# RemoteSensingTools/vSmartMOM.jl

Hardware: AMD Instinct MI355X
Metric: spectral-points/s (whole node) for rt_run, O2-A band (higher is better)
Workload: dtype f64; 1 GPU; C2: O2-A 759-770 nm, nStokes=3, Nquad=20 (N=60), 40 layers, 10000 spectral points/GPU, m=0..2, Rayleigh+synthetic O2 absorption, Lambertian 0.15; ranks=1, collective_backend=none (1 rank), N=60, layers=40, points_per_gpu=10000, fourier_moments=3

## Files before the change

### include/vsmartmom_hip.h

```cpp
#ifndef VSMARTMOM_HIP_H
#define VSMARTMOM_HIP_H

#include <stddef.h>
#include <stdint.h>

#ifdef __cplusplus
extern "C" {
#endif

typedef enum vsm_status {
  VSM_OK = 0,
  VSM_ERR_INVALID_ARG = 1,
  VSM_ERR_UNSUPPORTED = 2,
  VSM_ERR_HIP = 3,
  VSM_ERR_NO_DEVICE = 4
} vsm_status;

typedef enum vsm_iface {
  VSM_IFACE_00 = 0,
  VSM_IFACE_01 = 1,
  VSM_IFACE_10 = 2,
  VSM_IFACE_11 = 3
} vsm_iface;

// ... 336 lines not shown
size_t vsm_run_workspace_bytes_f32(int N, int n_stokes, int S, int nm, const int* coupling_h);
int vsm_run_create_f64(const vsm_quad_f64* q, int S, int nm, const int* m_h, const int* coupling_h, void* workspace,
                       size_t workspace_bytes, vsm_run** run);
int vsm_run_create_f32(const vsm_quad_f32* q, int S, int nm, const int* m_h, const int* coupling_h, void* workspace,
                       size_t workspace_bytes, vsm_run** run);
int vsm_run_create_ex_f64(const vsm_quad_f64* q, int S, int nm, const int* m_h, const int* coupling_h, void* workspace,
                          size_t workspace_bytes, unsigned flags, vsm_run** run);
int vsm_run_create_ex_f32(const vsm_quad_f32* q, int S, int nm, const int* m_h, const int* coupling_h, void* workspace,
                          size_t workspace_bytes, unsigned flags, vsm_run** run);
int vsm_run_create_view_f64(const vsm_quad_f64* q, int S, int nm, const int* m_h, const int* coupling_h, void* workspace,
                            size_t workspace_bytes, unsigned flags, int nrows, const int* rows_h, vsm_run** run);
int vsm_run_create_view_f32(const vsm_quad_f32* q, int S, int nm, const int* m_h, const int* coupling_h, void* workspace,
                            size_t workspace_bytes, unsigned flags, int nrows, const int* rows_h, vsm_run** run);
int vsm_run_create_view_f64(const vsm_quad_f64* q, int S, int nm, const int* m_h, const int* coupling_h, void* workspace,
                            size_t workspace_bytes, unsigned flags, int nrows, const int* rows_h, vsm_run** run);
int vsm_run_create_view_f32(const vsm_quad_f32* q, int S, int nm, const int* m_h, const int* coupling_h, void* workspace,
                            size_t workspace_bytes, unsigned flags, int nrows, const int* rows_h, vsm_run** run);
int vsm_run_layer_f64(vsm_run* run, int ndoubl, const double* dtau, const double* varpi, const double* tau_sum,
                      const double* F0, int ncomp, const double* const* Zpp, const double* const* Zmp, long long z_stride,
                      const double* fcomp, int toa, const int* layer_coupling_h, void* stream);
int vsm_run_layer_f32(vsm_run* run, int ndoubl, const float* dtau, const float* varpi, const float* tau_sum,
                      const float* F0, int ncomp, const float* const* Zpp, const float* const* Zmp, long long z_stride,
                      const float* fcomp, int toa, const int* layer_coupling_h, void* stream);
int vsm_run_export_f64(vsm_run* run, const vsm_composite_f64* comps, void* stream);
int vsm_run_export_f32(vsm_run* run, const vsm_composite_f32* comps, void* stream);
int vsm_run_import_f64(vsm_run* run, const vsm_composite_f64* comps, void* stream);
int vsm_run_import_f32(vsm_run* run, const vsm_composite_f32* comps, void* stream);
int vsm_run_zw_tail(vsm_run* run);
int vsm_run_view_rows(vsm_run* run, int nrows, const int* rows_h);
int vsm_run_view_block(const vsm_run* run, int block, int* im, int* n, int* nv, int* local_rows);
int vsm_run_view_rows(vsm_run* run, int nrows, const int* rows_h);
int vsm_run_view_block(const vsm_run* run, int block, int* im, int* n, int* nv, int* local_rows);
int vsm_run_destroy(vsm_run* run);
int vsm_stokes_coupling_f64(int N, int n_stokes, int nblocks, const double* Zpp, const double* Zmp, int* mask_d, void* stream);
int vsm_stokes_coupling_f32(int N, int n_stokes, int nblocks, const float* Zpp, const float* Zmp, int* mask_d, void* stream);

typedef struct vsm_added_rs_f64 {
  double *ier_mp, *iet_pp, *ier_pm, *iet_mm;
  double *ieJ0_p, *ieJ0_m;
  int K;
  int reserved;
} vsm_added_rs_f64;
typedef struct vsm_added_rs_f32 {
  float *ier_mp, *iet_pp, *ier_pm, *iet_mm;
  float *ieJ0_p, *ieJ0_m;
  int K;
// ... 174 lines not shown
```

### vsmartmom.jl_amd/_lib.py

```python
from __future__ import annotations

import ctypes as C
import os

_HERE = os.path.dirname(os.path.abspath(__file__))
LIB_PATH = os.environ.get("VSM_LIB_PATH") or os.path.join(_HERE, "lib", "libvsmartmom_hip.so")


class VSMError(RuntimeError):
    pass


class vsm_quad_f64(C.Structure):
    _fields_ = [("mu", C.c_void_p), ("wt", C.c_void_p), ("N", C.c_int), ("n_stokes", C.c_int),
                ("i_mu0", C.c_int), ("mu0", C.c_double)]


class vsm_quad_f32(C.Structure):
    _fields_ = [("mu", C.c_void_p), ("wt", C.c_void_p), ("N", C.c_int), ("n_stokes", C.c_int),
                ("i_mu0", C.c_int), ("mu0", C.c_float)]


class vsm_added(C.Structure):
    _fields_ = [("r_mp", C.c_void_p), ("t_pp", C.c_void_p), ("r_pm", C.c_void_p), ("t_mm", C.c_void_p),
# ... 104 lines not shown
    "vsm_doubling_inelastic_work_elems": (_SZ, [_I, _I, _I]),
    "vsm_interaction_inelastic_work_elems": (_SZ, [_I, _I, _I]),
    "vsm_elemental_inelastic_rrs_{T}": (_I, [_P, _I, _I, _I, _P, _P, _P, _P, _P, _P]),
    "vsm_doubling_inelastic_rrs_{T}": (_I, [_I, _I, _I, _I, _P, _P, _P, _P, _P, _P]),
    "vsm_interaction_inelastic_rrs_{T}": (_I, [_I, _I, _I, _P, _P, _P, _P, _P, _P, _P]),
    "vsm_copy_added_to_composite_ie_{T}": (_I, [_I, _I, _P, _P, _P]),
    "vsm_postprocess_vza_ie_{T}": (_I, [_I, _I, _I, _I, _I, _P, _P, _P, _P, _P, _P, _P]),
    "vsm_ss_column_{T}": (_I, [_P, _I, _I, _I, _P, _P, _P, _P, _P, _P, _P, _P, _P, _P, _I, _P, _P, _P, _P, _P, _P, _P]),
    "vsm_ss_column_lin_{T}": (_I, [_P, _I, _I, _I, _I, _I, _I, _I, _I, _P, _P, _P, _P, _P, _P, _P, _P, _P, _P, _I, _P, _P, _P, _P, _P, _P, _P,
                                   _P, _P, _I, _P, _P, _P, _P, _P]),
    "vsm_ss_column_rrs_{T}": (_I, [_P, _I, _I, _I, _I, _P, _P, _P, _P, _P, _P, _P, _P, _I, _I, _P, _P, _P, _P, _P]),
    "vsm_exact_ss_path1_{T}": (_I, [_I, _I, _I, _I, _I, _P, _P, _P, _P, "{R}", _P, _P, _P]),
    "vsm_exact_ss_path2_{T}": (_I, [_I, _I, _I, _I, _I, _P, _P, _I, _P, "{R}", _P, _P, _P]),
    "vsm_exact_ss_path34_{T}": (_I, [_I, _I, _I, _I, _I, _P, _P, _P, _P, _P, _P, _P, _P, "{R}", _P, _P, _P, _P]),
    "vsm_exact_ss_jac12_{T}": (_I, [_I, _I, _I, _I, _I, _P, _P, _P, _P, _I, _P, "{R}", _P, _P, _P, _P, _P, _P, _P]),
    "vsm_run_supported": (_I, [_I, _I, _I]),
    "vsm_run_workspace_bytes": (_SZ, [_I, _I, _I, _I, _P]),
    "vsm_run_supported_f32": (_I, [_I, _I, _I]),
    "vsm_run_workspace_bytes_f32": (_SZ, [_I, _I, _I, _I, _P]),
    "vsm_run_create_{T}": (_I, [_P, _I, _I, _P, _P, _P, _SZ, _P]),
    "vsm_run_create_ex_{T}": (_I, [_P, _I, _I, _P, _P, _P, _SZ, C.c_uint, _P]),
    "vsm_run_create_view_{T}": (_I, [_P, _I, _I, _P, _P, _P, _SZ, C.c_uint, _I, _P, _P]),
    "vsm_run_layer_{T}": (_I, [_P, _I, _P, _P, _P, _P, _I, _P, _P, _LL, _P, _I, _P, _P]),
    "vsm_run_export_{T}": (_I, [_P, _P, _P]),
    "vsm_run_import_{T}": (_I, [_P, _P, _P]),
    "vsm_run_zw_tail": (_I, [_P]),
    "vsm_run_view_rows": (_I, [_P, _I, _P]),
    "vsm_run_view_block": (_I, [_P, _I, _P, _P, _P, _P]),
    "vsm_run_destroy": (_I, [_P]),
    "vsm_stokes_coupling_{T}": (_I, [_I, _I, _I, _P, _P, _P, _P]),
    "vsm_level_radiance_work_elems": (_SZ, [_I, _I]),
    "vsm_level_radiance_{T}": (_I, [_I, _I, _I, _I, _P, _P, _P, _P, _P, _LL, _P, _P, _P, _P, _P, _P, _P]),
    "vsm_level_radiance_oplevel_{T}": (_I, [_I, _I, _I, _I, _P, _P, _P, _P, _P, _LL, _P, _P, _P, _P, _P, _P, _P]),
    "vsm_level_radiance_src_{T}": (_I, [_I, _I, _I, _I, _P, _P, _P, _I, _P, _P, _LL, _P, _P, _P, _P, _P, _P, _P]),
    "vsm_level_radiance_ie_{T}": (_I, [_I, _I, _I, _I, _P, _I, _P, _P, _P, _P, _LL, _P, _P, _P, _P, _P, _P, _P, _P, _P, _P, _P]),
    "vsm_level_radiance_lin_{T}": (_I, [_I, _I, _I, _I, _I, _I, _P, _P, _P, _P, _LL, _P, _P, _P, _LL, _P, _P, _LL, _LL, _P, _P, _P, _P, _P,
                                        _P]),
    "vsm_test_lds_mm_{T}": (_I, [_I, _I, _P, _P, _P, _P]),
    "vsm_test_lds_inv_{T}": (_I, [_I, _I, _P, _P, _I, _P, _P]),
    "vsm_test_poison_lds": (_I, [_P]),
}


def exported_symbols():
    out = []
    for name in _SIGS:
# ... 91 lines not shown
```

### vsmartmom.jl_amd/core_rt.py

```python
from __future__ import annotations

import ctypes as C
import dataclasses
import math
import os
from dataclasses import dataclass
from typing import List, Optional

import numpy as np
import torch

from . import _lib
from . import host_model as H
from .architectures import GPU, CPU, architecture, array_type, devi, synchronize_if_gpu, to_host

IFACE = {"00": 0, "01": 1, "10": 2, "11": 3}
MOMENT_BATCH = 4
MOMENT_BATCH_MAX = 24
MOMENT_BATCHING = True
THERMAL_FUSION = True
NATIVE_RUN = True
NATIVE_SOURCES_ONLY = True
NATIVE_VIEW_ROWS = True
VIEW_ROWS_MAX = 16
NATIVE_ZW_TAIL = True
NATIVE_DROPIN = True
REFERENCE_ORDER = False


def _require_gpu(arch):
    if not isinstance(arch, GPU):
        raise _lib.VSMError("vsmartmom.jl_amd provides the MI355X path only; architecture %r has no compute path here "
                            "(no CPU fallback by design)" % (arch,))
    if not torch.cuda.is_available():
        raise _lib.VSMError("no MI355X visible to HIP (torch.cuda.is_available() is False)")
    if arch.device_index != torch.cuda.current_device():
        raise _lib.VSMError("architecture GPU(%d) is not the current HIP device (%d): one process per GPU -- call "
                            "torch.cuda.set_device(%d) first" % (arch.device_index, torch.cuda.current_device(),
                                                                 arch.device_index))


def _torch_dtype(FT):
    return torch.float64 if np.dtype(FT) == np.float64 else torch.float32


def _stream_ptr():
    return C.c_void_p(torch.cuda.current_stream().cuda_stream)

# ... 246 lines not shown

_work_cache = {}


def layer_forward_multi_(tau_sum, dtau, F0, props_list, ms, ndoubl: int, dq: DeviceQuad, toa: bool, comps, added: AddedLayer):
    nm = len(ms)
    p0 = props_list[0]
    q, a = dq.cstruct(), added.cstruct()
    dtype = comps[0].dtype
    carr = (type(comps[0].cstruct()) * nm)(*[c.cstruct() for c in comps])
    marr = (C.c_int * nm)(*[int(m) for m in ms])
    zpp = (C.c_void_p * nm)(*[p.Zpp.data_ptr() for p in props_list])
    zmp = (C.c_void_p * nm)(*[p.Zmp.data_ptr() for p in props_list])
    ncomp = 0 if p0.fcomp is None else int(p0.fcomp.shape[1])
    _lib.call("vsm_layer_forward_multi", dtype, C.byref(q), comps[0].nSpec, nm, marr, ndoubl, _ptr(dtau), _ptr(p0.varpi),
              _ptr(tau_sum), _ptr(F0), ncomp, zpp, zmp, 0 if ncomp else p0.z_stride, _ptr(p0.fcomp), None, 1 if toa else 0,
              carr, C.byref(a), _stream_ptr())


def run_layer_native_(run, nm: int, ndoubl: int, dtau, varpi, tau_sum, F0, ncomp: int, zpp, zmp, z_stride: int, fcomp, toa: bool,
                      layer_coupling=None, dtype=torch.float64):
    _lib.call("vsm_run_layer", dtype, run, ndoubl, _ptr(dtau), _ptr(varpi), _ptr(tau_sum), _ptr(F0), ncomp, zpp, zmp, z_stride,
              _ptr(fcomp), 1 if toa else 0, layer_coupling, _stream_ptr())


def interaction_(scattering_interface: str, comp: CompositeLayer, added: AddedLayer, oplevel: bool = False,
                 work: Optional[torch.Tensor] = None):
    a, c = added.cstruct(), comp.cstruct()
    N, S = comp.N, comp.nSpec
    fused = (scattering_interface == "11" and not oplevel
             and N <= _lib.lib().vsm_fused_max_n(8 if comp.dtype == torch.float64 else 4))
    if not fused and work is None:
        key = (N, S, comp.dtype, str(comp.R_mp.device))
        work = _work_cache.get(key)
        if work is None:
            _work_cache.clear()
            work = _lib.poison(torch.empty(int(_lib.lib().vsm_interaction_work_elems(N, S)), dtype=comp.dtype, device=comp.R_mp.device))
            _work_cache[key] = work
    name = "vsm_interaction_oplevel" if oplevel else "vsm_interaction"
    _lib.call(name, comp.dtype, IFACE[scattering_interface], N, S, C.byref(c), C.byref(a), _ptr(work), _stream_ptr())


_phi_cache = {}


def brdf_azimuth_quadrature(arch, FT):
# ... 517 lines not shown
            return self.R_SFI, self.T_SFI
        self.added.j0_p.zero_()
        eps2 = 2 * np.finfo(FT).eps
        has_noscat = any(ly["props"].max_tau_varpi <= eps2 for ly in self.moments[0]["layers"])
        sequential = trace is not None or not MOMENT_BATCHING or has_noscat or REFERENCE_ORDER
        want = max(MOMENT_BATCH, min(MOMENT_BATCH_MAX, 4096 // max(self.S, 1)))
        nb = 1 if sequential else min(want, len(self.moments))
        while len(self._composites) < nb:
            self._composites.append(make_composite_layer(FT, self.arch, (self.N, self.N), self.S))
        native = self._native_moments() if trace is None and not has_noscat and not REFERENCE_ORDER else set()
        walk_src = streams is None and trace is None and not has_noscat
        if getattr(self, "_view_rows", None) is None:
            self._view_rows = view_rows_of(pol, model.vza, self.qp)
        view_rows = self._view_rows if streams is None else None
        for c in self._composites:
            c._sources_only = walk_src and REFERENCE_ORDER
            c._view_rows = view_rows if c._sources_only else None
        for g0 in range(0, len(self.moments), nb):
            group = self.moments[g0:g0 + nb]
            comps = self._composites[:len(group)]
            nat = [k for k in range(len(group)) if (g0 + k) in native]
            if nat:
                self._run_layers_native([group[k] for k in nat], [comps[k] for k in nat], sources_only=streams is None,
                                        view_rows=view_rows)
            rest = [k for k in range(len(group)) if (g0 + k) not in native]
            group_l, comps_l = [group[k] for k in rest], [comps[k] for k in rest]
            for iz in range(self.Nz if rest else 0):
                ly0 = group_l[0]["layers"][iz]
                if len(group_l) > 1 and ly0["props"].max_tau_varpi > eps2 and (iz == 0 or ly0["iface"] == "11"):
                    layer_forward_multi_(ly0["tau_sum"], ly0["dtau"], self.F0, [mom["layers"][iz]["props"] for mom in group_l],
                                         [mom["m"] for mom in group_l], ly0["nd"], self.dq, iz == 0, comps_l, self.added)
                    continue
                for mom, comp in zip(group_l, comps_l):
                    ly = mom["layers"][iz]
                    rt_kernel_(pol, self.added, comp, ly["props"], ly["iface"], ly["tau_sum"], mom["m"], self.dq,
                               self.arch, iz + 1, self.F0, FT, model.numerics, dtau=ly["dtau"], ndoubl=ly["nd"], trace=trace,
                               work=self.work, keep_added=has_noscat)
            for mom, comp in zip(group, comps):
                m = mom["m"]
                weight = FT(0.5 / math.pi) if m == 0 else FT(1.0 / math.pi)
                create_surface_layer_(model.surface, self.added_surface, m, self.dq, mom["tau_sum_surface"], rho=mom["rho"])
                interaction_(mom["iface_surface"], comp, self.added_surface, work=self.work)
                if self.compute_hdrf:
                    interaction_hdrf_(pol, comp, self.added_surface, m, self.dq, model.vza, model.vaz, self.qp, float(weight),
                                      self.hdr_J, self.hdr, self.bhr_uw, self.bhr_dw)
                postprocessing_vza_(pol, comp, model.vza, model.vaz, self.qp, m, float(weight), self.R_SFI, self.T_SFI)
                thermal_pass = self.thermal_B is not None and (m == 0 or (m == 1 and self._thermal_carry))
# ... 3 lines not shown
                    Jm, Jp = comp.J0_m.clone(), comp.J0_p.clone()
                    if thermal_pass:
                        Jm += self._th_comp.J0_m
                        Jp += self._th_comp.J0_p
                    streams.append(dict(m=m, weight=float(weight), R_mp=comp.R_mp.clone(), T_pp=comp.T_pp.clone(), J0_m=Jm, J0_p=Jp))
        for c in self._composites:
            c._sources_only = False
            c._view_rows = None
        if isinstance(model.surface, H.CoxMunkSurface) and self.ss_correction:
            apply_ss_correction_(self.R_SFI, model.surface, pol, model.vza, model.vaz, self.qp.mu0,
                                 self.moments[-1]["tau_sum_surface"], model.m_max, self.arch, FT)
        return self.R_SFI, self.T_SFI

    def _native_moments(self):
        if not NATIVE_RUN or getattr(self, "coupling", None) is None or not self.moments:
            return set()
        eps2 = 2 * np.finfo(self.FT).eps
        for iz, ly in enumerate(self.moments[0]["layers"]):
            p = ly["props"]
            if p.max_tau_varpi <= eps2 or (iz > 0 and ly["iface"] != "11") or (p.fcomp is not None and p.fcomp.shape[1] > 4):
                return set()
        return {i for i, mom in enumerate(self.moments) if run_supported(self.dt, self.N, self.pol.n, int(self.coupling[mom["m"]]))}

    def _run_layers_native(self, group, comps, sources_only: bool = True, export_at=None, view_rows=None):
        L = _lib.lib()
        nm, N, S, ns = len(group), self.N, self.S, self.pol.n
        marr = (C.c_int * nm)(*[int(mom["m"]) for mom in group])
        carr = (C.c_int * nm)(*[int(self.coupling[mom["m"]]) for mom in group])
        nbytes = run_workspace_bytes(self.dt, N, ns, S, nm, carr)
        ws = getattr(self, "_native_ws", None)
        if ws is None or ws.numel() * 8 < nbytes:
            ws = self._native_ws = _lib.poison(torch.empty(max(nbytes // 8, 2), dtype=torch.float64, device=self.dev))
        q = self.dq.cstruct()
        run = C.c_void_p()
        run_create_(self.dt, q, S, nm, marr, carr, ws, nbytes, sources_only, view_rows, run)
        try:
            if NATIVE_ZW_TAIL and not torch.cuda.is_current_stream_capturing():
                _lib.check(L.vsm_run_zw_tail(run))
            for iz in range(self.Nz):
                ly0 = group[0]["layers"][iz]
                props = [mom["layers"][iz]["props"] for mom in group]
                p0 = props[0]
                zpp = (C.c_void_p * nm)(*[p.Zpp.data_ptr() for p in props])
                zmp = (C.c_void_p * nm)(*[p.Zmp.data_ptr() for p in props])
                ncomp = 0 if p0.fcomp is None else int(p0.fcomp.shape[1])
                lc = (C.c_int * nm)(*[self._layer_coupling(mom["m"], iz) for mom in group])
                run_layer_native_(run, nm, int(ly0["nd"]), ly0["dtau"], p0.varpi, ly0["tau_sum"], self.F0, ncomp, zpp, zmp,
                                  0 if ncomp else p0.z_stride, p0.fcomp, iz == 0, lc, self.dt)
                if export_at and (iz + 1) in export_at:
                    cc = (type(comps[0].cstruct()) * nm)(*[c.cstruct() for c in comps])
                    _lib.call("vsm_run_export", self.dt, run, cc, _stream_ptr())
                    export_at[iz + 1](comps)
            cc = (type(comps[0].cstruct()) * nm)(*[c.cstruct() for c in comps])
            _lib.call("vsm_run_export", self.dt, run, cc, _stream_ptr())
        finally:
            L.vsm_run_destroy(run)

    def _thermal_slot(self, mom, weight):
        self._thermal_begin(mom)
        comp = self._th_comp
        self._thermal_walk(mom, comp, 0, self.Nz)
        surf = self._thermal_surface(mom)
        interaction_(mom["iface_surface"], comp, surf, oplevel=True, work=self.work)
        postprocessing_vza_(self.pol, comp, self.model.vza, self.model.vaz, self.qp, mom["m"], weight, self.R_SFI, self.T_SFI)

    def _thermal_begin(self, mom):
        N, S, FT = self.N, self.S, self.FT
        if getattr(self, "_th_added", None) is None:
            self._th_added = make_added_layer(FT, self.arch, (N, N), S, d_symmetric=0)
            self._th_surf = make_added_layer(FT, self.arch, (N, N), S, shared=not self.spectral_surface)
            self._th_comp = make_composite_layer(FT, self.arch, (N, N), S)
            self._th_F0 = torch.zeros_like(self.F0)
            self._th_ones = torch.ones(max(S, 1), dtype=self.dt, device=self.dev)
        if mom["m"] == 0:
            eps2 = 2 * np.finfo(FT).eps
# ... 41 lines not shown
                    zero_added_noscat_(added, props.tau, self.dq)
                    added.j0_p.zero_()
                    added.j0_m.zero_()
                if iz == first:
                    copy_added_to_composite_(comp, added)
                else:
                    interaction_(ly["iface"], comp, added, oplevel=True, work=self.work)
            if after and (iz + 1) in after:
                after[iz + 1](comp)

    def _thermal_surface(self, mom):
        create_surface_layer_(self.model.surface, self._th_surf, mom["m"], self.dq, mom["tau_sum_surface"], rho=mom["rho"])
        self._th_surf.j0_p.zero_()
        self._th_surf.j0_m.zero_()
        return self._th_surf

    def run_graph(self):
        if getattr(self, "_graph", None) is None:
            if self.added.d_symmetric == 0 or any(ly["props"].fcomp is not None for ly in self.moments[0]["layers"]):
                raise _lib.VSMError("run_graph(): only scenes that run entirely in the fused layer kernels (every layer "
                                    "scattering, N within the on-chip limit, one scatterer per layer) can be captured")
            gs = torch.cuda.Stream()
            gs.wait_stream(torch.cuda.current_stream())
            with torch.cuda.stream(gs):
                self.run()
            torch.cuda.synchronize()
            g = torch.cuda.CUDAGraph()
            with torch.cuda.graph(g, stream=gs):
                self.run()
            self._graph, self._graph_stream = g, gs
        self._graph.replay()
        return self.R_SFI, self.T_SFI

    def results_host(self):
        return to_host(self.R_SFI).transpose(2, 1, 0).copy(), to_host(self.T_SFI).transpose(2, 1, 0).copy()

    def results_host_full(self):
        R, T = self.results_host()
        return (R, T, np.zeros_like(R), np.zeros_like(T), to_host(self.hdr).transpose(2, 1, 0).copy(),
                to_host(self.bhr_uw)[:, 0].copy(), to_host(self.bhr_dw)[:, 0].copy())

    def flops_per_point(self) -> float:
        N = float(self.N)
        tot = 0.0
        for mom in self.moments:
            for iz, ly in enumerate(mom["layers"]):
                tot += ly["nd"] * (12 * N ** 3 + 8 * N ** 2)
                if iz > 0:
                    tot += 24 * N ** 3 + 8 * N ** 2
            tot += 24 * N ** 3 + 8 * N ** 2
        return tot

# ... 47 lines not shown
```

### vsmartmom.jl_amd/csrc/vsm_native.hip

```cpp
#include <stdlib.h>

#include <vector>

#include "vsm_native_dev.h"
#include "vsm_native_run.h"

#ifndef VSM_NATIVE_PARK_RT
#define VSM_NATIVE_PARK_RT 3
#endif

namespace vsm {

struct nlayer_comps {
  double* c[NSUB_MAX];
};

namespace {

template <int RT, int KS, int KZ = KS>
__device__ __forceinline__ void ned_body(nsmem<RT, (4 * KS + 2 > 16 * RT)>& sm, npos<RT>& p, int n, int gsz, unsigned uvmask, int ndoubl,
                                         const double* __restrict__ img, nstrip<RT>& r_s, nstrip<RT>& t_s, int* status) {
  using G = ngeo<RT>;
  constexpr unsigned dP = 0, dQ = G::AF * 8;
  double* jp = sm.vec[0];
// ... 1673 lines not shown
    map_view_rows(run);
  }
  run->ws = workspace;
  run->ws_elems = total;
  run->pure_diag.assign(run->subs.size(), 0);
  for (size_t i = 0; i < run->subs.size(); ++i) {
    const nat_sub& sb = run->subs[i];
    bool placed = false;
    for (auto& cl : run->classes) {
      const nat_sub& h = run->subs[cl[0]];
      if (h.n == sb.n && h.gsz == sb.gsz && h.uvmask == sb.uvmask && (int)cl.size() < NSUB_MAX) {
        cl.push_back((int)i);
        placed = true;
        break;
      }
    }
    if (!placed) run->classes.push_back(std::vector<int>{(int)i});
  }
  *run_out = run;
  return VSM_OK;
}

template <typename T>
static int run_layer(vsm_run* run, int ndoubl, const T* dtau, const T* varpi, const T* tau_sum, const T* F0, int ncomp,
                     const T* const* Zpp, const T* const* Zmp, long long z_stride, const T* fcomp, int toa,
                     const int* layer_coupling, void* stream) {
  VSM_REQUIRE(run && dtau && varpi && tau_sum && F0 && Zpp && Zmp, "vsm_run_layer: null argument");
  VSM_REQUIRE(run->elem_size == (int)sizeof(T), "vsm_run_layer: the run was created for %d-byte arrays", run->elem_size);
  VSM_REQUIRE(ndoubl >= 0 && ndoubl < 60 && ncomp >= 0 && ncomp <= 4 && (ncomp == 0 || fcomp), "vsm_run_layer: bad ndoubl / component mix");
  ++run->layers;
  if (run->S == 0) return VSM_OK;
  hipStream_t st = as_stream(stream);
  int* status = device_status();
  if (!status) return VSM_ERR_HIP;
  const quad<T> q = run_quad<T>(run);
  auto trivial = [&](const nat_sub& sb) {
    if (!layer_coupling || layer_coupling[sb.im] < 0) return false;
    for (int a = 0; a < sb.gsz; ++a)
      for (int b = 0; b < sb.gsz; ++b)
        if ((layer_coupling[sb.im] >> (4 * sb.g[a] + sb.g[b])) & 1) return false;
    return true;
  };
  {
    nguard_args<T> ga;
    for (int k = 0; k < NSUB_MAX; ++k) {
      const int im = k < run->nm ? k : 0;
      VSM_REQUIRE(Zpp[im] && Zmp[im], "vsm_run_layer: null Z of moment %d", im);
      ga.zp[k] = Zpp[im];
      ga.zm[k] = Zmp[im];
      ga.allowed[k] = 0;
    }
    for (const nat_sub& sb : run->subs) {
      if (trivial(sb)) continue;
      for (int a = 0; a < sb.gsz; ++a)
        for (int b = 0; b < sb.gsz; ++b) ga.allowed[sb.im] |= 1u << (4 * sb.g[a] + sb.g[b]);
    }
    const int nmat = ncomp ? ncomp : (z_stride ? run->S : 1);
    hipLaunchKernelGGL((k_coupling_guard<T>), dim3(nmat, run->nm), dim3(256), 0, st, run->N, run->ns,
                       ncomp ? (long long)run->N * run->N : z_stride, ga, status);
    VSM_LAUNCH_CHECK("k_coupling_guard");
  }
  T* const ws = static_cast<T*>(run->ws);
  const int src = (run->flags & VSM_RUN_SOURCES_ONLY) ? 1 : 0;
  const int view = (run->flags & VSM_RUN_VIEW_ROWS) ? 1 : 0;
  size_t pre_total = 0;
  for (const nat_sub& sb : run->subs)
    if (!trivial(sb)) pre_total += pre_stride_rt(sb.rt) * (size_t)run->S;
  T* pre = nullptr;
  if (pre_total) {
    pre = static_cast<T*>(scratch(pre_total * sizeof(T), 3, st));
    if (!pre) return VSM_ERR_HIP;
  }
  size_t off = 0;
  for (const auto& cl : run->classes) {
    const nat_sub& h = run->subs[cl[0]];
    std::vector<int> act, triv[3];
    for (int i : cl) {
      if (!trivial(run->subs[i])) {
        act.push_back(i);
        run->pure_diag[i] = 0;
      } else if (toa) {
        triv[1].push_back(i);
        run->pure_diag[i] = 1;
      } else {
        triv[run->pure_diag[i] ? 2 : 0].push_back(i);
      }
    }
    for (int mode = 0; mode < 3; ++mode) {
      if (triv[mode].empty()) continue;
      ndiag_args<T> da;
      const int nt = (int)triv[mode].size();
      for (int k = 0; k < NSUB_MAX; ++k) {
        const nat_sub& sb = run->subs[triv[mode][k < nt ? k : 0]];
        da.comp[k] = ws + sb.comp_off;
        da.gsz[k] = sb.gsz;
        da.g0[k] = sb.g[0] | (sb.g[1] << 4) | (sb.g[2] << 8) | (sb.g[3] << 12);
      }
      hipLaunchKernelGGL((k_native_diag_layer<T>), dim3(run->S, nt), dim3(256), 0, st, q, h.rt, h.n, (T)ldexp(1.0, ndoubl), mode,
                         src, view, dtau, da, view ? view_of(run, triv[mode]) : nview{});
      VSM_LAUNCH_CHECK("k_native_diag_layer");
    }
    const int nsub = (int)act.size();
    if (!nsub) continue;
    npre_args<T> pa;
    T* lc[NSUB_MAX];
    for (int k = 0; k < NSUB_MAX; ++k) {
      const nat_sub& sb = run->subs[act[k < nsub ? k : 0]];
      pa.s[k].m = sb.m;
      pa.s[k].gsz = sb.gsz;
      for (int a = 0; a < 4; ++a) pa.s[k].g[a] = sb.g[a];
      VSM_REQUIRE(Zpp[sb.im] && Zmp[sb.im], "vsm_run_layer: null Z of moment %d", sb.im);
      pa.s[k].z = zsrc<T>{Zpp[sb.im], Zmp[sb.im], ncomp ? 0 : z_stride, ncomp, fcomp};
      lc[k] = ws + sb.comp_off;
    }
    T* pre_cl = pre + off;
    off += pre_stride_rt(h.rt) * (size_t)run->S * nsub;
    native_launch_pre(h.rt, ncomp > 0, q, run->S, nsub, h.n, ndoubl, dtau, varpi, tau_sum, F0, pa, pre_cl, st);
    VSM_LAUNCH_CHECK("k_elemental_native");
    const nview vw = view ? view_of(run, act) : nview{};
    const int rc = native_launch_layer(h, run->S, nsub, ndoubl, toa, src, pre_cl, lc, status, view ? &vw : nullptr, st);
    if (rc) return rc;
  }
  return VSM_OK;
}

template <typename T, typename CS, bool IMPORT>
static int run_convert(vsm_run* run, const CS* comps, void* stream) {
  VSM_REQUIRE(run && comps, "vsm_run_export / import: null argument");
  VSM_REQUIRE(run->elem_size == (int)sizeof(T), "vsm_run_export / import: the run was created for %d-byte arrays", run->elem_size);
  if (IMPORT) ++run->imports;
  if (run->S == 0) return VSM_OK;
  if (IMPORT) {
    run->pure_diag.assign(run->subs.size(), 0);
    run->flags &= ~(unsigned)VSM_RUN_ZW_TAIL;
    for (nat_sub& sb : run->subs) sb.kz = sb.ks;
  }
  for (int im = 0; im < run->nm; ++im) {
    const CS& c = comps[im];
    VSM_REQUIRE(c.R_mp && c.R_pm && c.T_pp && c.T_mm && c.J0_p && c.J0_m, "vsm_run_export / import: null composite array (moment %d)", im);
    const composite<T> cc{c.R_mp, c.R_pm, c.T_pp, c.T_mm, c.J0_p, c.J0_m};
    const ngroup_map<T> gm = group_map<T>(run, im);
    const int view = (run->flags & VSM_RUN_VIEW_ROWS) ? 1 : 0;
    const nview vw = view ? view_of_moment(run, im) : nview{};
    if (IMPORT)
      hipLaunchKernelGGL((k_native_import<T>), dim3(run->S), dim3(256), 0, as_stream(stream), run->N, run->ns, view, gm, vw, cc);
    else
// ... 84 lines not shown
  run->view_rows.assign(rows, rows + nrows);
  map_view_rows(run);
  return VSM_OK;
}

int vsm_run_view_block(const vsm_run* run, int block, int* im, int* n, int* nv, int* local_rows) {
  VSM_REQUIRE(run && im && n && nv && local_rows, "vsm_run_view_block: null argument");
  VSM_REQUIRE(block >= 0 && block < (int)run->subs.size(), "vsm_run_view_block: the run has %d blocks", (int)run->subs.size());
  const nat_sub& sb = run->subs[block];
  *im = sb.im;
  *n = sb.n;
  *nv = (run->flags & VSM_RUN_VIEW_ROWS) ? sb.nv : 0;
  for (int v = 0; v < *nv; ++v) local_rows[v] = sb.vrow[v];
  return VSM_OK;
}

int vsm_run_zw_tail(vsm_run* run) {
  VSM_REQUIRE(run, "vsm_run_zw_tail: null argument");
  VSM_REQUIRE(run->layers == 0, "vsm_run_zw_tail: the run has taken layer steps already");
  return run->elem_size == 8 ? zw_tail<double>(run) : VSM_OK;
}

int vsm_run_destroy(vsm_run* run) {
  delete run;
  return VSM_OK;
}

int vsm_run_layer_f64(vsm_run* run, int ndoubl, const double* dtau, const double* varpi, const double* tau_sum, const double* F0,
                      int ncomp, const double* const* Zpp, const double* const* Zmp, long long z_stride, const double* fcomp,
                      int toa, const int* layer_coupling, void* stream) {
  return run_layer<double>(run, ndoubl, dtau, varpi, tau_sum, F0, ncomp, Zpp, Zmp, z_stride, fcomp, toa, layer_coupling, stream);
}
int vsm_run_layer_f32(vsm_run* run, int ndoubl, const float* dtau, const float* varpi, const float* tau_sum, const float* F0,
                      int ncomp, const float* const* Zpp, const float* const* Zmp, long long z_stride, const float* fcomp,
                      int toa, const int* layer_coupling, void* stream) {
  return run_layer<float>(run, ndoubl, dtau, varpi, tau_sum, F0, ncomp, Zpp, Zmp, z_stride, fcomp, toa, layer_coupling, stream);
}

int vsm_run_export_f64(vsm_run* run, const vsm_composite_f64* comps, void* stream) {
  return run_convert<double, vsm_composite_f64, false>(run, comps, stream);
}
int vsm_run_export_f32(vsm_run* run, const vsm_composite_f32* comps, void* stream) {
  return run_convert<float, vsm_composite_f32, false>(run, comps, stream);
}
int vsm_run_import_f64(vsm_run* run, const vsm_composite_f64* comps, void* stream) {
  return run_convert<double, vsm_composite_f64, true>(run, comps, stream);
}
int vsm_run_import_f32(vsm_run* run, const vsm_composite_f32* comps, void* stream) {
  return run_convert<float, vsm_composite_f32, true>(run, comps, stream);
}

int vsm_stokes_coupling_f64(int N, int n_stokes, int nblocks, const double* Zpp, const double* Zmp, int* mask_d, void* stream) {
  return stokes_coupling<double>(N, n_stokes, nblocks, Zpp, Zmp, mask_d, stream);
}
int vsm_stokes_coupling_f32(int N, int n_stokes, int nblocks, const float* Zpp, const float* Zmp, int* mask_d, void* stream) {
  return stokes_coupling<float>(N, n_stokes, nblocks, Zpp, Zmp, mask_d, stream);
}

}
// ... 3 lines not shown
```

### vsmartmom.jl_amd/csrc/vsm_native_run.h

```cpp
#pragma once
#include <vector>

#include "vsm_internal.h"

namespace vsm {

constexpr int NSUB_MAX = VSM_MM_MAX;

struct nat_sub {
  int im;
  int m;
  int gsz, g[4];
  unsigned uvmask;
  int n, rt, ks;
  int kz;
  size_t comp_off;
  int nv;
  int vrow[VSM_RUN_VIEW_MAX];
};

struct nview {
  int nv[NSUB_MAX];
  unsigned pk[NSUB_MAX][VSM_RUN_VIEW_MAX / 4];
  __host__ __device__ int row(int k, int v) const { return (int)((pk[k][v >> 2] >> (8 * (v & 3))) & 255u); }
// ... 2 lines not shown
    for (int v = 0; v < nv[k]; ++v) at = row(k, v) == r ? v : at;
    return at;
  }
};

}

struct vsm_run {
  const void *mu, *wt;
  int N, ns, i_mu0;
  double mu0;
  int elem_size;
  int S, nm;
  unsigned flags;
  std::vector<int> view_rows;
  std::vector<int> m;
  std::vector<vsm::nat_sub> subs;
  std::vector<std::vector<int>> classes;
  void* ws;
  size_t ws_elems;
  int layers = 0;
  int imports = 0;
  std::vector<char> pure_diag;
};

namespace vsm {

constexpr int NATIVE_MAX_ROWS = 96;
constexpr int NATIVE32_MAX_ROWS = 128;

constexpr int rt_of(int n) {
  const int ks = (n + 3) / 4;
  return (ks % 4 == 0 && ks >= 4) ? ks / 4 : (4 * ks + 2 + 15) / 16;
}
constexpr size_t comp_stride_rt(int rt) { return (size_t)4 * (16 * rt) * (16 * rt) + 2 * 16 * rt; }
constexpr size_t pre_stride_rt(int rt) { return (size_t)2 * (16 * rt) * (16 * rt) + 3 * 16 * rt; }

template <typename T>
struct nsub_pre {
  int m, gsz;
  int g[4];
  zsrc<T> z;
};
template <typename T>
struct npre_args {
  nsub_pre<T> s[NSUB_MAX];
// ... 10 lines not shown
```

Before: 26510 spectral-points/s.

## Add batched column API that pipelines elemental pre-pass and layer kernels across streams

Adds vsm_run_column, which takes every layer of a column in one host call instead of one ctypes call per layer. It launches the elemental pre-pass on a dedicated stream into double-buffered scratch rings per class, and runs the layer kernels of different classes on up to two chain streams, synchronised with events. The aim is to cut per-layer Python/ctypes overhead and to let layer N+1's pre computation overlap layer N's adding/doubling kernels. In exchange it adds extra streams, events and scratch memory, and the path is switched off when exporting, under graph capture, or when the layer function has been monkeypatched.

```diff
diff --git a/include/vsmartmom_hip.h b/include/vsmartmom_hip.h
--- a/include/vsmartmom_hip.h
+++ b/include/vsmartmom_hip.h
@@ -382,6 +382,14 @@
 int vsm_run_layer_f32(vsm_run* run, int ndoubl, const float* dtau, const float* varpi, const float* tau_sum,
                       const float* F0, int ncomp, const float* const* Zpp, const float* const* Zmp, long long z_stride,
                       const float* fcomp, int toa, const int* layer_coupling_h, void* stream);
+int vsm_run_column_f64(vsm_run* run, int nlayers, const int* ndoubl_h, const double* const* dtau_h, const double* const* varpi_h,
+                       const double* const* tau_sum_h, const double* F0, const int* ncomp_h, const double* const* Zpp_h,
+                       const double* const* Zmp_h, const long long* z_stride_h, const double* const* fcomp_h, const int* toa_h,
+                       const int* layer_coupling_h, void* stream);
+int vsm_run_column_f32(vsm_run* run, int nlayers, const int* ndoubl_h, const float* const* dtau_h, const float* const* varpi_h,
+                       const float* const* tau_sum_h, const float* F0, const int* ncomp_h, const float* const* Zpp_h,
+                       const float* const* Zmp_h, const long long* z_stride_h, const float* const* fcomp_h, const int* toa_h,
+                       const int* layer_coupling_h, void* stream);
 int vsm_run_export_f64(vsm_run* run, const vsm_composite_f64* comps, void* stream);
 int vsm_run_export_f32(vsm_run* run, const vsm_composite_f32* comps, void* stream);
 int vsm_run_import_f64(vsm_run* run, const vsm_composite_f64* comps, void* stream);
diff --git a/vsmartmom.jl_amd/_lib.py b/vsmartmom.jl_amd/_lib.py
--- a/vsmartmom.jl_amd/_lib.py
+++ b/vsmartmom.jl_amd/_lib.py
@@ -150,6 +150,7 @@
     "vsm_run_create_ex_{T}": (_I, [_P, _I, _I, _P, _P, _P, _SZ, C.c_uint, _P]),
     "vsm_run_create_view_{T}": (_I, [_P, _I, _I, _P, _P, _P, _SZ, C.c_uint, _I, _P, _P]),
     "vsm_run_layer_{T}": (_I, [_P, _I, _P, _P, _P, _P, _I, _P, _P, _LL, _P, _I, _P, _P]),
+    "vsm_run_column_{T}": (_I, [_P, _I, _P, _P, _P, _P, _P, _P, _P, _P, _P, _P, _P, _P, _P]),
     "vsm_run_export_{T}": (_I, [_P, _P, _P]),
     "vsm_run_import_{T}": (_I, [_P, _P, _P]),
     "vsm_run_zw_tail": (_I, [_P]),
diff --git a/vsmartmom.jl_amd/core_rt.py b/vsmartmom.jl_amd/core_rt.py
--- a/vsmartmom.jl_amd/core_rt.py
+++ b/vsmartmom.jl_amd/core_rt.py
@@ -24,6 +24,7 @@
 NATIVE_VIEW_ROWS = True
 VIEW_ROWS_MAX = 16
 NATIVE_ZW_TAIL = True
+NATIVE_COLUMN = True
 NATIVE_DROPIN = True
 REFERENCE_ORDER = False
 
@@ -316,6 +317,21 @@
                       layer_coupling=None, dtype=torch.float64):
     _lib.call("vsm_run_layer", dtype, run, ndoubl, _ptr(dtau), _ptr(varpi), _ptr(tau_sum), _ptr(F0), ncomp, zpp, zmp, z_stride,
               _ptr(fcomp), 1 if toa else 0, layer_coupling, _stream_ptr())
+
+
+_run_layer_native_lib = run_layer_native_
+
+
+def run_column_native_(run, nm: int, layers, F0, dtype=torch.float64):
+    n = len(layers)
+    ints = lambda k, ct=C.c_int: (ct * n)(*[int(ly[k]) for ly in layers])
+    ptrs = lambda k: (C.c_void_p * n)(*[_ptr(ly[k]).value for ly in layers])
+    flat = lambda k: (C.c_void_p * (n * nm))(*[ly[k][i] for ly in layers for i in range(nm)])
+    lc = None
+    if all(ly[10] is not None for ly in layers):
+        lc = (C.c_int * (n * nm))(*[int(ly[10][i]) for ly in layers for i in range(nm)])
+    _lib.call("vsm_run_column", dtype, run, n, ints(0), ptrs(1), ptrs(2), ptrs(3), _ptr(F0), ints(4), flat(5), flat(6),
+              ints(7, C.c_longlong), ptrs(8), ints(9), lc, _stream_ptr())
 
 
 def interaction_(scattering_interface: str, comp: CompositeLayer, added: AddedLayer, oplevel: bool = False,
@@ -879,7 +895,7 @@
             nat = [k for k in range(len(group)) if (g0 + k) in native]
             if nat:
                 self._run_layers_native([group[k] for k in nat], [comps[k] for k in nat], sources_only=streams is None,
-                                        view_rows=view_rows)
+                                        view_rows=view_rows, column=streams is None)
             rest = [k for k in range(len(group)) if (g0 + k) not in native]
             group_l, comps_l = [group[k] for k in rest], [comps[k] for k in rest]
             for iz in range(self.Nz if rest else 0):
@@ -929,7 +945,7 @@
                 return set()
         return {i for i, mom in enumerate(self.moments) if run_supported(self.dt, self.N, self.pol.n, int(self.coupling[mom["m"]]))}
 
-    def _run_layers_native(self, group, comps, sources_only: bool = True, export_at=None, view_rows=None):
+    def _run_layers_native(self, group, comps, sources_only: bool = True, export_at=None, view_rows=None, column: bool = False):
         L = _lib.lib()
         nm, N, S, ns = len(group), self.N, self.S, self.pol.n
         marr = (C.c_int * nm)(*[int(mom["m"]) for mom in group])
@@ -944,6 +960,9 @@
         try:
             if NATIVE_ZW_TAIL and not torch.cuda.is_current_stream_capturing():
                 _lib.check(L.vsm_run_zw_tail(run))
+            column = (column and NATIVE_COLUMN and not export_at and run_layer_native_ is _run_layer_native_lib
+                      and not getattr(self, "_graph_walk", False) and not torch.cuda.is_current_stream_capturing())
+            steps = []
             for iz in range(self.Nz):
                 ly0 = group[0]["layers"][iz]
                 props = [mom["layers"][iz]["props"] for mom in group]
@@ -952,12 +971,18 @@
                 zmp = (C.c_void_p * nm)(*[p.Zmp.data_ptr() for p in props])
                 ncomp = 0 if p0.fcomp is None else int(p0.fcomp.shape[1])
                 lc = (C.c_int * nm)(*[self._layer_coupling(mom["m"], iz) for mom in group])
+                if column:
+                    steps.append((int(ly0["nd"]), ly0["dtau"], p0.varpi, ly0["tau_sum"], ncomp, zpp, zmp,
+                                  0 if ncomp else p0.z_stride, p0.fcomp, iz == 0, lc))
+                    continue
                 run_layer_native_(run, nm, int(ly0["nd"]), ly0["dtau"], p0.varpi, ly0["tau_sum"], self.F0, ncomp, zpp, zmp,
                                   0 if ncomp else p0.z_stride, p0.fcomp, iz == 0, lc, self.dt)
                 if export_at and (iz + 1) in export_at:
                     cc = (type(comps[0].cstruct()) * nm)(*[c.cstruct() for c in comps])
                     _lib.call("vsm_run_export", self.dt, run, cc, _stream_ptr())
                     export_at[iz + 1](comps)
+            if steps:
+                run_column_native_(run, nm, steps, self.F0, self.dt)
             cc = (type(comps[0].cstruct()) * nm)(*[c.cstruct() for c in comps])
             _lib.call("vsm_run_export", self.dt, run, cc, _stream_ptr())
         finally:
@@ -1045,12 +1070,16 @@
                                     "scattering, N within the on-chip limit, one scatterer per layer) can be captured")
             gs = torch.cuda.Stream()
             gs.wait_stream(torch.cuda.current_stream())
-            with torch.cuda.stream(gs):
-                self.run()
-            torch.cuda.synchronize()
-            g = torch.cuda.CUDAGraph()
-            with torch.cuda.graph(g, stream=gs):
-                self.run()
+            self._graph_walk = True
+            try:
+                with torch.cuda.stream(gs):
+                    self.run()
+                torch.cuda.synchronize()
+                g = torch.cuda.CUDAGraph()
+                with torch.cuda.graph(g, stream=gs):
+                    self.run()
+            finally:
+                self._graph_walk = False
             self._graph, self._graph_stream = g, gs
         self._graph.replay()
         return self.R_SFI, self.T_SFI
diff --git a/vsmartmom.jl_amd/csrc/vsm_native.hip b/vsmartmom.jl_amd/csrc/vsm_native.hip
--- a/vsmartmom.jl_amd/csrc/vsm_native.hip
+++ b/vsmartmom.jl_amd/csrc/vsm_native.hip
@@ -1,5 +1,6 @@
 #include <stdlib.h>
 
+#include <algorithm>
 #include <vector>
 
 #include "vsm_native_dev.h"
@@ -1719,106 +1720,262 @@
 }
 
 template <typename T>
-static int run_layer(vsm_run* run, int ndoubl, const T* dtau, const T* varpi, const T* tau_sum, const T* F0, int ncomp,
-                     const T* const* Zpp, const T* const* Zmp, long long z_stride, const T* fcomp, int toa,
-                     const int* layer_coupling, void* stream) {
-  VSM_REQUIRE(run && dtau && varpi && tau_sum && F0 && Zpp && Zmp, "vsm_run_layer: null argument");
+struct nlayer_args {
+  int ndoubl;
+  const T *dtau, *varpi, *tau_sum, *F0;
+  int ncomp;
+  const T* const* Zpp;
+  const T* const* Zmp;
+  long long z_stride;
+  const T* fcomp;
+  int toa;
+  const int* layer_coupling;
+};
+
+template <typename T>
+static int check_layer(const vsm_run* run, const nlayer_args<T>& L) {
+  VSM_REQUIRE(run && L.dtau && L.varpi && L.tau_sum && L.F0 && L.Zpp && L.Zmp, "vsm_run_layer: null argument");
   VSM_REQUIRE(run->elem_size == (int)sizeof(T), "vsm_run_layer: the run was created for %d-byte arrays", run->elem_size);
-  VSM_REQUIRE(ndoubl >= 0 && ndoubl < 60 && ncomp >= 0 && ncomp <= 4 && (ncomp == 0 || fcomp), "vsm_run_layer: bad ndoubl / component mix");
+  VSM_REQUIRE(L.ndoubl >= 0 && L.ndoubl < 60 && L.ncomp >= 0 && L.ncomp <= 4 && (L.ncomp == 0 || L.fcomp),
+              "vsm_run_layer: bad ndoubl / component mix");
+  return VSM_OK;
+}
+static int check_layer_Z(const vsm_run* run, const void* const* Zpp, const void* const* Zmp) {
+  for (int im = 0; im < run->nm; ++im) VSM_REQUIRE(Zpp[im] && Zmp[im], "vsm_run_layer: null Z of moment %d", im);
+  return VSM_OK;
+}
+
+template <typename T>
+static bool layer_trivial(const nlayer_args<T>& L, const nat_sub& sb) {
+  if (!L.layer_coupling || L.layer_coupling[sb.im] < 0) return false;
+  for (int a = 0; a < sb.gsz; ++a)
+    for (int b = 0; b < sb.gsz; ++b)
+      if ((L.layer_coupling[sb.im] >> (4 * sb.g[a] + sb.g[b])) & 1) return false;
+  return true;
+}
+
+template <typename T>
+static int launch_guard(const vsm_run* run, const nlayer_args<T>& L, int* status, hipStream_t st) {
+  nguard_args<T> ga;
+  for (int k = 0; k < NSUB_MAX; ++k) {
+    const int im = k < run->nm ? k : 0;
+    ga.zp[k] = L.Zpp[im];
+    ga.zm[k] = L.Zmp[im];
+    ga.allowed[k] = 0;
+  }
+  for (const nat_sub& sb : run->subs) {
+    if (layer_trivial(L, sb)) continue;
+    for (int a = 0; a < sb.gsz; ++a)
+      for (int b = 0; b < sb.gsz; ++b) ga.allowed[sb.im] |= 1u << (4 * sb.g[a] + sb.g[b]);
+  }
+  const int nmat = L.ncomp ? L.ncomp : (L.z_stride ? run->S : 1);
+  hipLaunchKernelGGL((k_coupling_guard<T>), dim3(nmat, run->nm), dim3(256), 0, st, run->N, run->ns,
+                     L.ncomp ? (long long)run->N * run->N : L.z_stride, ga, status);
+  VSM_LAUNCH_CHECK("k_coupling_guard");
+  return VSM_OK;
+}
+
+template <typename T>
+static size_t class_pre_elems(const vsm_run* run, const std::vector<int>& cl, const nlayer_args<T>& L) {
+  size_t n = 0;
+  for (int i : cl)
+    if (!layer_trivial(L, run->subs[i])) n += pre_stride_rt(run->subs[i].rt) * (size_t)run->S;
+  return n;
+}
+
+template <typename T>
+static int class_diag(vsm_run* run, const std::vector<int>& cl, const nlayer_args<T>& L, std::vector<int>& act, hipStream_t st) {
+  const nat_sub& h = run->subs[cl[0]];
+  T* const ws = static_cast<T*>(run->ws);
+  const int src = (run->flags & VSM_RUN_SOURCES_ONLY) ? 1 : 0;
+  const int view = (run->flags & VSM_RUN_VIEW_ROWS) ? 1 : 0;
+  std::vector<int> triv[3];
+  act.clear();
+  for (int i : cl) {
+    if (!layer_trivial(L, run->subs[i])) {
+      act.push_back(i);
+      run->pure_diag[i] = 0;
+    } else if (L.toa) {
+      triv[1].push_back(i);
+      run->pure_diag[i] = 1;
+    } else {
+      triv[run->pure_diag[i] ? 2 : 0].push_back(i);
+    }
+  }
+  for (int mode = 0; mode < 3; ++mode) {
+    if (triv[mode].empty()) continue;
+    ndiag_args<T> da;
+    const int nt = (int)triv[mode].size();
+    for (int k = 0; k < NSUB_MAX; ++k) {
+      const nat_sub& sb = run->subs[triv[mode][k < nt ? k : 0]];
+      da.comp[k] = ws + sb.comp_off;
+      da.gsz[k] = sb.gsz;
+      da.g0[k] = sb.g[0] | (sb.g[1] << 4) | (sb.g[2] << 8) | (sb.g[3] << 12);
+    }
+    hipLaunchKernelGGL((k_native_diag_layer<T>), dim3(run->S, nt), dim3(256), 0, st, run_quad<T>(run), h.rt, h.n,
+                       (T)ldexp(1.0, L.ndoubl), mode, src, view, L.dtau, da, view ? view_of(run, triv[mode]) : nview{});
+    VSM_LAUNCH_CHECK("k_native_diag_layer");
+  }
+  return VSM_OK;
+}
+
+template <typename T>
+static int class_pre(const vsm_run* run, const std::vector<int>& act, const nlayer_args<T>& L, T* pre_cl, hipStream_t st) {
+  const nat_sub& h = run->subs[act[0]];
+  const int nsub = (int)act.size();
+  npre_args<T> pa;
+  for (int k = 0; k < NSUB_MAX; ++k) {
+    const nat_sub& sb = run->subs[act[k < nsub ? k : 0]];
+    pa.s[k].m = sb.m;
+    pa.s[k].gsz = sb.gsz;
+    for (int a = 0; a < 4; ++a) pa.s[k].g[a] = sb.g[a];
+    pa.s[k].z = zsrc<T>{L.Zpp[sb.im], L.Zmp[sb.im], L.ncomp ? 0 : L.z_stride, L.ncomp, L.fcomp};
+  }
+  native_launch_pre(h.rt, L.ncomp > 0, run_quad<T>(run), run->S, nsub, h.n, L.ndoubl, L.dtau, L.varpi, L.tau_sum, L.F0, pa, pre_cl, st);
+  VSM_LAUNCH_CHECK("k_elemental_native");
+  return VSM_OK;
+}
+template <typename T>
+static int class_layer(const vsm_run* run, const std::vector<int>& act, const nlayer_args<T>& L, const T* pre_cl, int* status,
+                       hipStream_t st) {
+  const nat_sub& h = run->subs[act[0]];
+  const int nsub = (int)act.size();
+  T* const ws = static_cast<T*>(run->ws);
+  const int src = (run->flags & VSM_RUN_SOURCES_ONLY) ? 1 : 0;
+  const int view = (run->flags & VSM_RUN_VIEW_ROWS) ? 1 : 0;
+  T* lc[NSUB_MAX];
+  for (int k = 0; k < NSUB_MAX; ++k) lc[k] = ws + run->subs[act[k < nsub ? k : 0]].comp_off;
+  const nview vw = view ? view_of(run, act) : nview{};
+  return native_launch_layer(h, run->S, nsub, L.ndoubl, L.toa, src, pre_cl, lc, status, view ? &vw : nullptr, st);
+}
+
+template <typename T>
+static int run_layer(vsm_run* run, const nlayer_args<T>& L, void* stream) {
+  int rc = check_layer(run, L);
+  if (rc) return rc;
   ++run->layers;
   if (run->S == 0) return VSM_OK;
   hipStream_t st = as_stream(stream);
   int* status = device_status();
   if (!status) return VSM_ERR_HIP;
-  const quad<T> q = run_quad<T>(run);
-  auto trivial = [&](const nat_sub& sb) {
-    if (!layer_coupling || layer_coupling[sb.im] < 0) return false;
-    for (int a = 0; a < sb.gsz; ++a)
-      for (int b = 0; b < sb.gsz; ++b)
-        if ((layer_coupling[sb.im] >> (4 * sb.g[a] + sb.g[b])) & 1) return false;
-    return true;
-  };
-  {
-    nguard_args<T> ga;
-    for (int k = 0; k < NSUB_MAX; ++k) {
-      const int im = k < run->nm ? k : 0;
-      VSM_REQUIRE(Zpp[im] && Zmp[im], "vsm_run_layer: null Z of moment %d", im);
-      ga.zp[k] = Zpp[im];
-      ga.zm[k] = Zmp[im];
-      ga.allowed[k] = 0;
-    }
-    for (const nat_sub& sb : run->subs) {
-      if (trivial(sb)) continue;
-      for (int a = 0; a < sb.gsz; ++a)
-        for (int b = 0; b < sb.gsz; ++b) ga.allowed[sb.im] |= 1u << (4 * sb.g[a] + sb.g[b]);
-    }
-    const int nmat = ncomp ? ncomp : (z_stride ? run->S : 1);
-    hipLaunchKernelGGL((k_coupling_guard<T>), dim3(nmat, run->nm), dim3(256), 0, st, run->N, run->ns,
-                       ncomp ? (long long)run->N * run->N : z_stride, ga, status);
-    VSM_LAUNCH_CHECK("k_coupling_guard");
-  }
-  T* const ws = static_cast<T*>(run->ws);
-  const int src = (run->flags & VSM_RUN_SOURCES_ONLY) ? 1 : 0;
-  const int view = (run->flags & VSM_RUN_VIEW_ROWS) ? 1 : 0;
+  if ((rc = check_layer_Z(run, (const void* const*)L.Zpp, (const void* const*)L.Zmp))) return rc;
+  if ((rc = launch_guard(run, L, status, st))) return rc;
   size_t pre_total = 0;
-  for (const nat_sub& sb : run->subs)
-    if (!trivial(sb)) pre_total += pre_stride_rt(sb.rt) * (size_t)run->S;
+  for (const auto& cl : run->classes) pre_total += class_pre_elems(run, cl, L);
   T* pre = nullptr;
   if (pre_total) {
     pre = static_cast<T*>(scratch(pre_total * sizeof(T), 3, st));
     if (!pre) return VSM_ERR_HIP;
   }
   size_t off = 0;
+  std::vector<int> act;
   for (const auto& cl : run->classes) {
-    const nat_sub& h = run->subs[cl[0]];
-    std::vector<int> act, triv[3];
-    for (int i : cl) {
-      if (!trivial(run->subs[i])) {
-        act.push_back(i);
-        run->pure_diag[i] = 0;
-      } else if (toa) {
-        triv[1].push_back(i);
-        run->pure_diag[i] = 1;
-      } else {
-        triv[run->pure_diag[i] ? 2 : 0].push_back(i);
-      }
-    }
-    for (int mode = 0; mode < 3; ++mode) {
-      if (triv[mode].empty()) continue;
-      ndiag_args<T> da;
-      const int nt = (int)triv[mode].size();
-      for (int k = 0; k < NSUB_MAX; ++k) {
-        const nat_sub& sb = run->subs[triv[mode][k < nt ? k : 0]];
-        da.comp[k] = ws + sb.comp_off;
-        da.gsz[k] = sb.gsz;
-        da.g0[k] = sb.g[0] | (sb.g[1] << 4) | (sb.g[2] << 8) | (sb.g[3] << 12);
-      }
-      hipLaunchKernelGGL((k_native_diag_layer<T>), dim3(run->S, nt), dim3(256), 0, st, q, h.rt, h.n, (T)ldexp(1.0, ndoubl), mode,
-                         src, view, dtau, da, view ? view_of(run, triv[mode]) : nview{});
-      VSM_LAUNCH_CHECK("k_native_diag_layer");
-    }
-    const int nsub = (int)act.size();
-    if (!nsub) continue;
-    npre_args<T> pa;
-    T* lc[NSUB_MAX];
-    for (int k = 0; k < NSUB_MAX; ++k) {
-      const nat_sub& sb = run->subs[act[k < nsub ? k : 0]];
-      pa.s[k].m = sb.m;
-      pa.s[k].gsz = sb.gsz;
-      for (int a = 0; a < 4; ++a) pa.s[k].g[a] = sb.g[a];
-      VSM_REQUIRE(Zpp[sb.im] && Zmp[sb.im], "vsm_run_layer: null Z of moment %d", sb.im);
-      pa.s[k].z = zsrc<T>{Zpp[sb.im], Zmp[sb.im], ncomp ? 0 : z_stride, ncomp, fcomp};
-      lc[k] = ws + sb.comp_off;
-    }
+    if ((rc = class_diag(run, cl, L, act, st))) return rc;
+    if (act.empty()) continue;
     T* pre_cl = pre + off;
-    off += pre_stride_rt(h.rt) * (size_t)run->S * nsub;
-    native_launch_pre(h.rt, ncomp > 0, q, run->S, nsub, h.n, ndoubl, dtau, varpi, tau_sum, F0, pa, pre_cl, st);
-    VSM_LAUNCH_CHECK("k_elemental_native");
-    const nview vw = view ? view_of(run, act) : nview{};
-    const int rc = native_launch_layer(h, run->S, nsub, ndoubl, toa, src, pre_cl, lc, status, view ? &vw : nullptr, st);
+    off += class_pre_elems(run, cl, L);
+    if ((rc = class_pre(run, act, L, pre_cl, st))) return rc;
+    if ((rc = class_layer(run, act, L, pre_cl, status, st))) return rc;
+  }
+  return VSM_OK;
+}
+
+constexpr int COL_CHAINS = 2, COL_RING = 2;
+constexpr int COL_SLOT0 = 16;
+
+static int column_streams(vsm_run* run, int n) {
+  while ((int)run->col_streams.size() < n) {
+    hipStream_t s = nullptr;
+    VSM_HIP(hipStreamCreateWithFlags(&s, hipStreamNonBlocking));
+    run->col_streams.push_back(s);
+  }
+  return VSM_OK;
+}
+static int column_events(vsm_run* run, int n) {
+  while ((int)run->col_events.size() < n) {
+    hipEvent_t e = nullptr;
+    VSM_HIP(hipEventCreateWithFlags(&e, hipEventDisableTiming));
+    run->col_events.push_back(e);
+  }
+  return VSM_OK;
+}
+
+template <typename T>
+static int run_column(vsm_run* run, int nlayers, const int* ndoubl, const T* const* dtau, const T* const* varpi,
+                      const T* const* tau_sum, const T* F0, const int* ncomp, const T* const* Zpp, const T* const* Zmp,
+                      const long long* z_stride, const T* const* fcomp, const int* toa, const int* layer_coupling, void* stream) {
+  VSM_REQUIRE(run && nlayers >= 0, "vsm_run_column: null run / negative layer count");
+  if (nlayers == 0) return VSM_OK;
+  VSM_REQUIRE(ndoubl && dtau && varpi && tau_sum && F0 && ncomp && Zpp && Zmp && z_stride && toa, "vsm_run_column: null table");
+  const int nm = run->nm;
+  std::vector<nlayer_args<T>> Ls((size_t)nlayers);
+  for (int k = 0; k < nlayers; ++k) {
+    Ls[k] = nlayer_args<T>{ndoubl[k], dtau[k], varpi[k], tau_sum[k], F0, ncomp[k], Zpp + (size_t)k * nm, Zmp + (size_t)k * nm,
+                           z_stride[k], fcomp ? fcomp[k] : nullptr, toa[k], layer_coupling ? layer_coupling + (size_t)k * nm : nullptr};
+    int rc = check_layer(run, Ls[k]);
+    if (!rc) rc = check_layer_Z(run, (const void* const*)Ls[k].Zpp, (const void* const*)Ls[k].Zmp);
     if (rc) return rc;
   }
-  return VSM_OK;
+  run->layers += nlayers;
+  if (run->S == 0) return VSM_OK;
+  hipStream_t st = as_stream(stream);
+  int* status = device_status();
+  if (!status) return VSM_ERR_HIP;
+
+  const int nc = (int)run->classes.size();
+  std::vector<int> chain(nc, -1);
+  std::vector<T*> ring((size_t)nc * COL_RING, nullptr);
+  int nchain = 0;
+  for (int c = 0; c < nc; ++c) {
+    size_t most = 0;
+    for (const auto& L : Ls) most = std::max(most, class_pre_elems(run, run->classes[c], L));
+    if (!most) continue;
+    chain[c] = nchain++ % COL_CHAINS;
+    for (int r = 0; r < COL_RING; ++r)
+      if (!(ring[(size_t)c * COL_RING + r] = static_cast<T*>(scratch(most * sizeof(T), COL_SLOT0 + COL_RING * c + r, st))))
+        return VSM_ERR_HIP;
+  }
+  const int nstream = nchain ? 1 + std::min(nchain, COL_CHAINS) : 0;
+  int rc = column_streams(run, nstream);
+  if (!rc) rc = column_events(run, 1 + COL_CHAINS + 2 * COL_RING * nc);
+  if (rc) return rc;
+  const hipEvent_t* ev = run->col_events.data();
+  auto ready = [&](int c, int r) { return ev[1 + COL_CHAINS + 2 * (COL_RING * c + r)]; };
+  auto done = [&](int c, int r) { return ev[1 + COL_CHAINS + 2 * (COL_RING * c + r) + 1]; };
+  if (nstream) {
+    VSM_HIP(hipEventRecord(ev[0], st));
+    for (int j = 0; j < nstream; ++j) VSM_HIP(hipStreamWaitEvent(run->col_streams[j], ev[0], 0));
+  }
+  hipStream_t pre_st = nstream ? run->col_streams[0] : st;
+  auto walk = [&]() -> int {
+    std::vector<int> act, steps(nc, 0);
+    for (const auto& L : Ls) {
+      int rw = launch_guard(run, L, status, st);
+      if (rw) return rw;
+      for (int c = 0; c < nc; ++c) {
+        hipStream_t cs = chain[c] < 0 ? st : run->col_streams[1 + chain[c]];
+        if ((rw = class_diag(run, run->classes[c], L, act, cs))) return rw;
+        if (act.empty()) continue;
+        const int r = steps[c] % COL_RING;
+        T* pre_cl = ring[(size_t)c * COL_RING + r];
+        if (steps[c] >= COL_RING) VSM_HIP(hipStreamWaitEvent(pre_st, done(c, r), 0));
+        if ((rw = class_pre(run, act, L, pre_cl, pre_st))) return rw;
+        VSM_HIP(hipEventRecord(ready(c, r), pre_st));
+        VSM_HIP(hipStreamWaitEvent(cs, ready(c, r), 0));
+        if ((rw = class_layer(run, act, L, pre_cl, status, cs))) return rw;
+        VSM_HIP(hipEventRecord(done(c, r), cs));
+        ++steps[c];
+      }
+    }
+    return VSM_OK;
+  };
+  rc = walk();
+  for (int j = 1; j < nstream; ++j) {
+    hipError_t e = hipEventRecord(ev[j], run->col_streams[j]);
+    if (e == hipSuccess) e = hipStreamWaitEvent(st, ev[j], 0);
+    if (e != hipSuccess && !rc) rc = hip_fail(e, "vsm_run_column: join");
+  }
+  return rc;
 }
 
 template <typename T, typename CS, bool IMPORT>
@@ -1949,6 +2106,10 @@
 }
 
 int vsm_run_destroy(vsm_run* run) {
+  if (run) {
+    for (hipEvent_t e : run->col_events) (void)hipEventDestroy(e);
+    for (hipStream_t s : run->col_streams) (void)hipStreamDestroy(s);
+  }
   delete run;
   return VSM_OK;
 }
@@ -1956,12 +2117,26 @@
 int vsm_run_layer_f64(vsm_run* run, int ndoubl, const double* dtau, const double* varpi, const double* tau_sum, const double* F0,
                       int ncomp, const double* const* Zpp, const double* const* Zmp, long long z_stride, const double* fcomp,
                       int toa, const int* layer_coupling, void* stream) {
-  return run_layer<double>(run, ndoubl, dtau, varpi, tau_sum, F0, ncomp, Zpp, Zmp, z_stride, fcomp, toa, layer_coupling, stream);
+  return run_layer<double>(run, {ndoubl, dtau, varpi, tau_sum, F0, ncomp, Zpp, Zmp, z_stride, fcomp, toa, layer_coupling}, stream);
 }
 int vsm_run_layer_f32(vsm_run* run, int ndoubl, const float* dtau, const float* varpi, const float* tau_sum, const float* F0,
                       int ncomp, const float* const* Zpp, const float* const* Zmp, long long z_stride, const float* fcomp,
                       int toa, const int* layer_coupling, void* stream) {
-  return run_layer<float>(run, ndoubl, dtau, varpi, tau_sum, F0, ncomp, Zpp, Zmp, z_stride, fcomp, toa, layer_coupling, stream);
+  return run_layer<float>(run, {ndoubl, dtau, varpi, tau_sum, F0, ncomp, Zpp, Zmp, z_stride, fcomp, toa, layer_coupling}, stream);
+}
+int vsm_run_column_f64(vsm_run* run, int nlayers, const int* ndoubl, const double* const* dtau, const double* const* varpi,
+                       const double* const* tau_sum, const double* F0, const int* ncomp, const double* const* Zpp,
+                       const double* const* Zmp, const long long* z_stride, const double* const* fcomp, const int* toa,
+                       const int* layer_coupling, void* stream) {
+  return run_column<double>(run, nlayers, ndoubl, dtau, varpi, tau_sum, F0, ncomp, Zpp, Zmp, z_stride, fcomp, toa, layer_coupling,
+                            stream);
+}
+int vsm_run_column_f32(vsm_run* run, int nlayers, const int* ndoubl, const float* const* dtau, const float* const* varpi,
+                       const float* const* tau_sum, const float* F0, const int* ncomp, const float* const* Zpp,
+                       const float* const* Zmp, const long long* z_stride, const float* const* fcomp, const int* toa,
+                       const int* layer_coupling, void* stream) {
+  return run_column<float>(run, nlayers, ndoubl, dtau, varpi, tau_sum, F0, ncomp, Zpp, Zmp, z_stride, fcomp, toa, layer_coupling,
+                           stream);
 }
 
 int vsm_run_export_f64(vsm_run* run, const vsm_composite_f64* comps, void* stream) {
diff --git a/vsmartmom.jl_amd/csrc/vsm_native_run.h b/vsmartmom.jl_amd/csrc/vsm_native_run.h
--- a/vsmartmom.jl_amd/csrc/vsm_native_run.h
+++ b/vsmartmom.jl_amd/csrc/vsm_native_run.h
@@ -48,6 +48,8 @@
   int layers = 0;
   int imports = 0;
   std::vector<char> pure_diag;
+  std::vector<hipStream_t> col_streams;
+  std::vector<hipEvent_t> col_events;
 };
 
 namespace vsm {
```

After: 26470 spectral-points/s. No clear change (-0.2%).
